# skitzoid/Box2D-MT

Hardware: AMD Instinct MI355X
Metric: world steps/sec at 99858 bodies per GPU (BASELINE config 3: Tumbler 100k, CCD off; Step = collide + island solve + broad-phase + state read-back); for N > 1: container-steps/s = world steps/s x N containers in the one sharded world (higher is better)
Workload: dtype f32

## Files before the change

### box2d-mt_amd/csrc/b2d_scan.h

```cpp
#ifndef B2D_SCAN_H
#define B2D_SCAN_H

#include <hip/hip_runtime.h>
#include <stdint.h>

#define SCAN_THREADS 256
#define SCAN_ITEMS 4
#define SCAN_TILE (SCAN_THREADS * SCAN_ITEMS)
#define SCAN_CHAIN_MAX_TILES 256
#define SCAN_ITEMS_WIDE 16
#define SCAN_TILE_WIDE (SCAN_THREADS * SCAN_ITEMS_WIDE)

__device__ __forceinline__ int scanAdd(int a, int b) { return a + b; }
__device__ __forceinline__ int4 scanAdd(int4 a, int4 b) { return make_int4(a.x + b.x, a.y + b.y, a.z + b.z, a.w + b.w); }
__device__ __forceinline__ void scanZero(int& a) { a = 0; }
__device__ __forceinline__ void scanZero(int4& a) { a = make_int4(0, 0, 0, 0); }
__device__ __forceinline__ void scanStoreAgent(int* p, int v) { __hip_atomic_store(p, v, __ATOMIC_RELAXED, __HIP_MEMORY_SCOPE_AGENT); }
__device__ __forceinline__ int scanLoadAgent(const int* p) { return __hip_atomic_load(p, __ATOMIC_RELAXED, __HIP_MEMORY_SCOPE_AGENT); }
__device__ __forceinline__ void scanStoreAgent(int4* p, int4 v)
{
	typedef int i4 __attribute__((ext_vector_type(4)));
	i4 q;
	q.x = v.x; q.y = v.y; q.z = v.z; q.w = v.w;
	asm volatile("global_store_dwordx4 %0, %1, off sc1\n\ts_nop 1" :: "v"(p), "v"(q) : "memory");
// ... 348 lines not shown
			unsigned long long m = __ballot(valid && ((d >> b) & 1));
			peers &= ((d >> b) & 1) ? m : ~m;
		}
		if (!valid) peers = 0;
		unsigned long long lower = peers & ((1ull << lane) - 1ull);
		int rankInWave = __popcll(lower);
		const bool first = valid && lower == 0;
		const int groupSize = __popcll(peers);
		if (first) waveCount[wave][d] = groupSize;
		__syncthreads();
		int total = 0;
		if (valid)
		{
			int off = digitBase[d];
			for (int w = 0; w < wave; ++w) off += waveCount[w][d];
			int dst = off + rankInWave;
			keysOut[dst] = key;
			valsOut[dst] = valR[k];
			if (first) total = waveCount[0][d] + waveCount[1][d] + waveCount[2][d] + waveCount[3][d];
		}
		__syncthreads();
		if (first)
		{
			bool lowest = true;
			for (int w = 0; w < wave; ++w) lowest = lowest && waveCount[w][d] == 0;
			if (lowest) digitBase[d] += total;
		}
		__syncthreads();
		if (first) waveCount[wave][d] = 0;
		__syncthreads();
	}
}

#endif
```

### box2d-mt_amd/csrc/b2hip_api_callbacks.h

```cpp

int b2hip_set_contact_filter(b2hip_world* w, b2hip_should_collide_fn fn, void* user)
{
	if (int rcu = checkUsable(w, "b2hip_set_contact_filter", true)) return rcu;
	w->filterFn = fn;
	w->filterUser = user;
	w->dw.userFilter = hasFilter(w) ? 1 : 0;
	return B2HIP_OK;
}

int b2hip_set_contact_filter_batch(b2hip_world* w, b2hip_should_collide_batch_fn fn, void* user)
{
	if (int rcu = checkUsable(w, "b2hip_set_contact_filter_batch", true)) return rcu;
	w->filterBatchFn = fn;
	if (fn) w->filterUser = user;
	w->dw.userFilter = hasFilter(w) ? 1 : 0;
	return B2HIP_OK;
}

int b2hip_default_should_collide(b2hip_world* w, int fixture_a, int fixture_b)
{
	if (!w || fixture_a < 0 || fixture_b < 0 || fixture_a >= (int)w->fixtures.size() || fixture_b >= (int)w->fixtures.size())
		return setError(B2HIP_ERR_INVALID, "bad fixture id");
	const HostFixture& a = w->fixtures[fixture_a];
	const HostFixture& b = w->fixtures[fixture_b];
// ... 154 lines not shown
	HIP_TRY(hipStreamSynchronize(w->stream));
	const void* src = nullptr;
	size_t elem = 16;
	switch (which)
	{
	case 0: src = w->b_pos.p; break;
	case 1: src = w->b_vel.p; break;
	case 2: src = w->li_bodies.p; elem = 4; break;
	case 3: src = w->b_force.p; break;
	case 4: src = w->b_flags.p; elem = 4; break;
	case 5: src = w->b_damp.p; break;
	case 6: src = w->b_mass.p; break;
	case 7: src = w->d_state.p; elem = 4; break;
	case 8: src = w->dbgPreVel.p; break;
	case 9: src = w->dbgVel.p; break;
	case 10: src = w->dbgLi.p; elem = 4; break;
	case 11: src = w->gridBar.p; elem = 4; break;
	case 12:
	{
		if (first < 0 || count < 0 || first + count > COLOR_SLOT_PADDED) return setError(B2HIP_ERR_INVALID, "colour census: [0, 65)");
		HIP_TRY(hipStreamSynchronize(w->stream));
		if (count > 0) HIP_TRY(hipMemcpy2D(out, sizeof(int), w->colorCount.p + colorSlot(first), COLOR_SLOT_STRIDE * sizeof(int), sizeof(int), (size_t)count, hipMemcpyDeviceToHost));
		return 0;
	}
	case 13: src = w->bodyColorMask.p; elem = 8; break;
	case 14: src = w->deg.p; elem = 4; break;
	case 15: src = w->hubList.p; elem = 4; break;
	case 16: src = w->bodyActive.p; elem = 8; break;
	case 17: src = w->b_blk1.p; elem = 4; break;
	case 18: src = w->li_ref.p; break;
	case 19: src = w->rowColor.p; elem = 4; break;
	case 20: src = w->blkRowStart.p; elem = 4; break;
	case 21: src = w->bodyRest.p; elem = 8; break;
	default: return setError(B2HIP_ERR_INVALID, "bad array id");
	}
	HIP_TRY(hipMemcpy(out, (const char*)src + (size_t)first * elem, (size_t)count * elem, hipMemcpyDeviceToHost));
	return 0;
}

int b2hip_debug_trace(b2hip_world* w, int index, char* label, int label_cap, uint64_t* hash)
{
	if (!w) return setError(B2HIP_ERR_INVALID, "null world");
	if (index < 0 || index >= (int)w->trace.size()) return 1;
	if (label && label_cap > 0)
	{
		strncpy(label, w->trace[index].first.c_str(), (size_t)label_cap - 1);
		label[label_cap - 1] = 0;
	}
	if (hash) *hash = w->trace[index].second;
	return 0;
}

int b2hip_get_profile(b2hip_world* w, float ms[13])
{
	if (!w || !ms) return setError(B2HIP_ERR_INVALID, "null argument");
	memcpy(ms, w->profile, sizeof(float) * 13);
	return 0;
}

int b2hip_get_counters(b2hip_world* w, b2hip_counters* out)
{
	if (!w || !out) return setError(B2HIP_ERR_INVALID, "null argument");
	memset(out, 0, sizeof(*out));
	out->bodies = (int)w->bodies.size();
	out->proxies = (int)w->fixtures.size();
	out->contacts = w->last.nContacts;
	out->touching_contacts = w->last.nTouching;
	out->islands = w->last.nIslands;
	out->small_islands = w->last.nSIslands;
	out->large_islands = w->last.nLIslands;
// ... 86 lines not shown
```

### box2d-mt_amd/csrc/b2hip_api_world.h

```cpp


const char* b2hip_last_error(void)
{
	return g_lastError.c_str();
}

const char* b2hip_version(void)
{
	return "b2hip 0.1 (gfx950)";
}

int b2hip_world_create(const b2hip_world_def* def, b2hip_world** out)
{
	if (!def || !out) return setError(B2HIP_ERR_INVALID, "null argument");
	int count = 0;
	hipError_t e = hipGetDeviceCount(&count);
	if (e != hipSuccess || count <= 0)
	{
		return setError(B2HIP_ERR_NO_DEVICE, "no HIP device available: the b2hip Step() path has no CPU fallback");
	}
	int current = 0;
	if (hipGetDevice(&current) != hipSuccess) current = 0;
	const int device = def->device >= 0 ? def->device : current;
	if (device >= count) return setError(B2HIP_ERR_NO_DEVICE, "no such HIP device");
// ... 166 lines not shown
	w->p_fat.release(); w->p_body.release(); w->p_shape.release(); w->p_key.release(); w->p_filter0.release(); w->p_filter1.release();
	w->p_mat.release(); w->d_shapes.release();
	for (int k = 0; k < 2; ++k)
	{
		w->c_ids[k].release(); w->c_key[k].release(); w->c_flags[k].release(); w->c_mat[k].release(); w->c_man0[k].release();
		w->c_man1[k].release(); w->c_imp[k].release(); w->c_man3[k].release(); w->c_color[k].release();
	}
	w->ht_keys.release(); w->d_joints.release(); w->d_gears.release(); w->li_ref.release();
	w->jadjStart.release(); w->jadj.release(); w->rootJointStart.release(); w->rootJointCursor.release();
	w->lj_list.release(); w->rootJointOkay.release();
	w->parent.release(); w->rootSeed.release(); w->rootBodies.release(); w->rootContacts.release(); w->rootJoints.release();
	w->rootIsland.release(); w->deg.release(); w->adjStart.release(); w->adjCursor.release(); w->adj.release(); w->adjSlot.release();
	w->rootScanIn.release(); w->rootScanOut.release();
	w->si_root.release(); w->si_bodyStart.release(); w->si_contactStart.release(); w->si_wStart.release(); w->si_maxLevel.release();
	w->si_bodies.release(); w->si_contacts.release(); w->si_level.release(); w->si_stack.release(); w->si_lastLevel.release();
	w->b_slot.release(); w->b_island.release(); w->chunkFirst.release();
	w->li_bodies.release(); w->li_contacts.release(); w->li_roots.release(); w->li_color.release(); w->colorCount.release();
	w->colorStart.release(); w->colorCursor.release(); w->li_sorted.release(); w->bodyClaim.release(); w->rootPen.release();
	w->bodyActive.release(); w->bodyRest.release(); w->b_posv.release(); w->evKey.release(); w->evInfo.release(); w->uncolList.release(); w->compactList.release(); w->gridBar.release(); w->hubRowOf.release(); w->hubList.release(); w->hubDelta.release(); w->hubMeta.release(); w->hubFirst.release(); w->solveSnapBody.release(); w->solveSnapImp.release(); w->solveSnapCFlags.release(); w->solveSnapJoints.release(); w->solveSnapGears.release();
	w->b_proxyHead.release(); w->p_next.release(); w->toiList.release(); w->toiPos2c.release(); w->toiDestroyList.release(); w->toiNewList.release();
	w->b_toiGroup.release(); w->toiGroups.release(); w->toiGroupCount.release(); w->toiGroupList.release(); w->toiMoved.release(); w->toiNew.release(); w->toiParent.release(); w->toiDomOf.release(); w->toiDomRoot.release(); w->toiDomCount.release(); w->toiDomBase.release(); w->toiDomFill.release(); w->toiDomFailed.release(); w->toiDomEvents.release(); w->toiDomList.release(); w->toiHull.release(); w->snapBody.release(); w->snapFat.release();
	w->c_mgr[0].release(); w->c_mgr[1].release(); w->dbgPreVel.release(); w->dbgVel.release(); w->dbgLi.release();
	w->rootSleepMin.release(); w->bodyColorMask.release(); w->rootDone.release(); w->lc.release(); w->warmDelta.release();
	w->moveBuf.release(); w->gridCount.release(); w->gridStart.release(); w->gridCursor.release(); w->gridItems.release(); w->gridFat.release(); w->arriveTree.release();
	w->largeProxies.release(); w->largeMoves.release(); w->pairKey.release(); w->pairKey2.release(); w->pairProxy.release(); w->pairProxy2.release();
	w->filterPairs.release();
	w->d_editOps.release();
	w->b_order.release(); w->orderBody.release(); w->bigRoots.release();
	w->pre_o0.release(); w->pre_o1.release(); w->pre_oimp.release(); w->pre_o3.release(); w->preRecs.release();
	w->postRecs.release(); w->filterList.release(); w->hostList.release(); w->toiLog.release(); w->toiVerdict.release();
	w->b_blk1.release(); w->b_adopt.release(); w->b_adoptStage.release(); w->blkRows.release(); w->blkRowStart.release(); w->blkCursor.release(); w->blkBodyCount.release(); w->blkBodyCursor.release();
	w->blkBodyStart.release(); w->blkBodies.release(); w->rowColor.release(); w->b_cutv.release();
	w->pairFirst.release(); w->pairRank.release(); w->scanTmp.release(); w->radixHist.release(); w->radixHistScan.release();
	w->keepFlag.release(); w->keepScan.release(); w->scanTmp4.release(); w->scanFlags.release(); w->stateOut.release(); w->consts.release();
	w->qIn.release(); w->qCounts.release(); w->qOffsets.release(); w->qItems.release(); w->qFlags.release(); w->qScanWork.release();
	w->qScanWords.release(); w->qWords.release(); w->qHits.release(); w->qDistances.release(); w->qPoses.release(); w->qShapes.release();
	w->qKeys.release(); w->qKeysWork.release(); w->qAny.release();
	if (w->qPinned) (void)hipHostFree(w->qPinned);
	if (w->h_state) (void)hipHostFree(w->h_state);
	if (w->h_dstate) (void)hipHostFree(w->h_dstate);
	if (w->h_pub) (void)hipHostFree(w->h_pub);
	if (w->h_pub2) (void)hipHostFree(w->h_pub2);
	if (w->h_solverWord) (void)hipHostFree(w->h_solverWord);
	for (int i = 0; i < 13; ++i)
		if (w->ev[i]) (void)hipEventDestroy(w->ev[i]);
	for (size_t i = 0; i < w->ktEvents.size(); ++i) (void)hipEventDestroy(w->ktEvents[i]);
	if (w->stream) (void)hipStreamDestroy(w->stream);
	if (w->stream2) (void)hipStreamDestroy(w->stream2);
	if (w->evFork) (void)hipEventDestroy(w->evFork);
	if (w->evJoin) (void)hipEventDestroy(w->evJoin);
	delete w;
}

int b2hip_set_gravity(b2hip_world* w, float gx, float gy)
{
	if (int rcu = checkUsable(w, "b2hip_set_gravity", true)) return rcu;
	if (!w) return setError(B2HIP_ERR_INVALID, "null world");
	w->def.gravity_x = gx;
	w->def.gravity_y = gy;
	return 0;
}

int b2hip_set_flags(b2hip_world* w, int allow_sleep, int warm_starting, int continuous, int sub_stepping)
{
	if (int rcu = checkUsable(w, "b2hip_set_flags", true)) return rcu;
	if (!w) return setError(B2HIP_ERR_INVALID, "null world");
	w->def.allow_sleep = allow_sleep;
// ... 1157 lines not shown
```

### box2d-mt_amd/csrc/b2hip_host_phases.h

```cpp

static int spExchangeState(b2hip_world* w, int mode);
static int spExchangePairs(b2hip_world* w, long long* totalPairs, int* straddling);
static int spResolve(b2hip_world* w, int nVirt = 0);
static int spAfterToi(b2hip_world* w);
static int spBeginStep(b2hip_world* w);

static int radixBits(int maxKey)
{
	int bits = 1;
	while ((1 << bits) <= maxKey && bits < 31) ++bits;
	return bits;
}

static void radixPasses(int first, int bits, std::vector<std::pair<int, int>>& out)
{
	const int passes = (bits + RADIX_BITS - 1) / RADIX_BITS;
	for (int p = 0, at = 0; p < passes; ++p)
	{
		const int width = (bits - at + (passes - p) - 1) / (passes - p);
		out.push_back(std::make_pair(first + at, width));
		at += width;
	}
}

static int radixSort(b2hip_world* w, uint64_t*& kin, uint64_t*& kout, int2*& vin, int2*& vout, const int* nPtr, int tilesCap, const std::vector<std::pair<int, int>>& passes, int overflowBit = 0)
{
	DW& d = w->dw;
	LAUNCH(w, k_radix_count, 1, 1, nPtr, 0, w->consts.p + 2, tilesCap, overflowBit ? &d.st->c.overflow : (int*)nullptr, overflowBit);
	for (size_t p = 0; p < passes.size(); ++p)
	{
		LAUNCH(w, k_radix_hist, tilesCap, RADIX_THREADS, kin, d.radixHist, nPtr, 0, passes[p].first, passes[p].second, tilesCap);
		deviceExclusiveScan<int>(w->stream, d.radixHist, w->radixHistScan.p, d.scanTmp, w->scanCtx, w->consts.p + 2, RADIX_DIGITS * tilesCap);
		LAUNCH(w, k_radix_scatter, tilesCap, RADIX_THREADS, kin, vin, kout, vout, w->radixHistScan.p, nPtr, 0, passes[p].first, passes[p].second);
		std::swap(kin, kout);
		std::swap(vin, vout);
	}
	return 0;
}

template <typename K>
static int applyHostList(b2hip_world* w, K kernel, const std::vector<int>& list)
{
	if (list.empty()) return 0;
	HIP_TRY(hipMemcpyAsync(w->hostList.p, list.data(), list.size() * sizeof(int), hipMemcpyHostToDevice, w->stream));
	LAUNCH(w, kernel, gridFor(list.size()), 256, w->dw, (const int*)w->hostList.p, (int)list.size());
	HIP_TRY(hipStreamSynchronize(w->stream));
	return 0;
}

static void askFilter(b2hip_world* w, const std::vector<int>& pairs2, std::vector<int>& verdict)
{
	const int n = (int)pairs2.size() / 2;
	verdict.assign((size_t)n, 1);
	if (n == 0) return;
	if (w->filterBatchFn) w->filterBatchFn(w->filterUser, n, pairs2.data(), verdict.data());
	else for (int i = 0; i < n; ++i) verdict[i] = w->filterFn(w->filterUser, pairs2[2 * i], pairs2[2 * i + 1]) ? 1 : 0;
}

static int userFilterPairs(b2hip_world* w, const int2* proxies)
{
// ... 1360 lines not shown
```

### box2d-mt_amd/csrc/b2hip_host_world.h

```cpp

static thread_local std::string g_lastError;

static int setError(int code, const std::string& msg)
{
	g_lastError = msg;
	return code;
}

#define HIP_TRY(expr)                                                                                   \
	do                                                                                                  \
	{                                                                                                   \
		hipError_t _e = (expr);                                                                         \
		if (_e != hipSuccess)                                                                           \
		{                                                                                               \
			return setError(B2HIP_ERR_HIP, std::string(#expr) + ": " + hipGetErrorString(_e));          \
		}                                                                                               \
	} while (0)

static void (*g_rcclDestroy)(void* comm) = nullptr;

template <typename T>
struct DevArray
{
	T* p = nullptr;
// ... 179 lines not shown
	int spIdle[6] = {0, 0, 0, 0, 0, 0};
	DevArray<int> spStraddle, spCount, spTarget, spSend, spRecv;
	std::vector<uint8_t> spOwners;
	bool spOwnersDirty = false;
	float spBounds[SHARD_MAX_RANKS + 1] = {0};
	b2hip_all_gather_fn gatherFn = nullptr;
	void* gatherUser = nullptr;
	int* spHost = nullptr;
	const int* spSendWiped = nullptr;
	int* spHdrHost = nullptr;
	int* spHdrDev = nullptr;
	int spHdrSeq = 0;
	int* spOwnHost = nullptr;
	int* spOwnDev = nullptr;
	size_t spOwnCapRows = 0;
	size_t spHostWords = 0;
	int spPairCap = 2048, spToiBodyCap = 256, spToiProxyCap = 512;
	int spOwned[SHARD_MAX_RANKS] = {0}, spOwnedProxies[SHARD_MAX_RANKS] = {0};
	long long spMigratedTotal = 0, spResolves = 0, spPairsSent = 0;
	size_t spBytesStep = 0;
	int spContactsBeforeToi = 0, spToiOrderBefore = 0, spTailCap = 64;
	int spToiUnsafe = 0;
	bool spToiSettled = false;
	DevArray<int4> spTailKey;
	DevArray<int2> spVirt;
	bool spTapeRecord = false;
	std::vector<std::pair<int*, size_t> > spTape;
	b2hip_world* spTapeFrom = nullptr;
	size_t spTapeCursor = 0;
	long long spToiRedos = 0;
	size_t spUp = 0;
	DevArray<int> scanFlags;
	ScanFlags scanCtx;
	DevArray<float> stateOut;
	DevArray<int> gridBar;
	int dfEpoch;
	bool noSideStream, profileDetail;
	int collideStage = -1;
	int solidRoundsEnv = 0;
	int collideSplitEnv = -1;
	bool collideUniOff = false;
	int collideSortEnv = -1;
	hipStream_t stream2 = nullptr;
	hipEvent_t evFork = nullptr, evJoin = nullptr;
	DevArray<int> consts;
	DevArray<unsigned long long> filterPairs;
	std::vector<int> nonStatic;
	bool orderDirty = false;
	DevArray<int> b_order, orderBody;
	DevArray<int> bigRoots;
	std::vector<int2> editOps;
	std::vector<int> proxyEdits;
	std::vector<int> fatEdits;
	bool proxyListsStale = false;
	DevArray<int2> d_editOps;
	b2hip_should_collide_fn filterFn = nullptr;
	void* filterUser = nullptr;
	bool refilterPending = false;
	b2hip_pre_solve_fn preSolveFn = nullptr;
	b2hip_pre_solve_batch_fn preSolveBatchFn = nullptr;
	b2hip_should_collide_batch_fn filterBatchFn = nullptr;
	void* preSolveUser = nullptr;
	bool postSolveOn = false;
	std::vector<b2hip_contact_impulse> postSolve;
	DevArray<float4> pre_o0, pre_o1, pre_oimp;
	DevArray<int4> pre_o3;
// ... 440 lines not shown
static int awaitColors(b2hip_world* w)
{
	if (int rc = pollPublished(w, (volatile const int*)&w->h_pub2->pubSeq, w->pubSeq2, "colour state")) return rc;
	memcpy(w->h_dstate, w->h_pub2, offsetof(DState, pubSeq));
	return 0;
}

static int awaitCensus(b2hip_world* w)
{
	if (w->pollDelayUs > 0) std::this_thread::sleep_for(std::chrono::microseconds(w->pollDelayUs));
	if (int rc = pollPublished(w, (volatile const int*)&w->h_pub->pubSeq, w->pubSeq, "island census")) return rc;
	memcpy(w->h_dstate, w->h_pub, offsetof(DState, pubSeq));
	return 0;
}

static bool envSet(const char* k) { return getenv(k) != nullptr; }
static bool envOn(const char* k) { const char* e = getenv(k); return e && atoi(e); }
static int envInt(const char* k, int unset) { const char* e = getenv(k); return e ? atoi(e) : unset; }

static void readSwitches(b2hip_world* w)
{
	DW& d = w->dw;
	w->debugSync = envSet("B2HIP_DEBUG");
	w->traceLaunches = envSet("B2HIP_TRACE_LAUNCHES");
	w->debugTrace = envSet("B2HIP_TRACE");
	w->forceLarge = envInt("B2HIP_FORCE_LARGE", 0);
	w->kernelTimingLaunches = envSet("B2HIP_SOLVER_LAUNCHES");
	w->noSideStream = envSet("B2HIP_NO_SIDE_STREAM");
	w->profileDetail = envInt("B2HIP_PROFILE_DETAIL", 1) != 0;
	if (const char* e = getenv("B2HIP_SOLID_ROUNDS")) { const int v = atoi(e); w->solidRoundsEnv = (v == 1 || v == 2 || v == 4 || v == 8) ? v : 0; }
	w->collideSplitEnv = envInt("B2HIP_COLLIDE_SPLIT", -1);
	w->collideUniOff = envInt("B2HIP_COLLIDE_UNI", 1) == 0;
	w->collideSortEnv = envInt("B2HIP_COLLIDE_SORT", -1);
	w->collideStage = envInt("B2HIP_COLLIDE_STAGE", -1);
	w->noSweepBlocks = envSet("B2HIP_NO_SWEEP_BLOCKS");
	w->tracePartition = envSet("B2HIP_TRACE_PARTITION");
	w->traceRecovery = envSet("B2HIP_TRACE_RECOVERY");
	if (const char* e = getenv("B2HIP_GRID_HALF")) { w->gridForced = true; w->gridHalf = atoi(e) != 0; d.gridHalf = w->gridHalf ? 1 : 0; }
	d.noChainCreate = envSet("B2HIP_TOI_NO_CHAIN_CREATE") ? 1 : 0;
	d.noOwnIdBlocks = envSet("B2HIP_NO_OWN_ID_BLOCKS") ? 1 : envSet("B2HIP_OWN_ID_BLOCKS_ALL") ? -1 : 0;
	w->noBlocks = envSet("B2HIP_NO_BLOCKS");
	w->blockLanes = 0;
	if (const char* e = getenv("B2HIP_BLOCK_LANES")) w->blockLanes = atoi(e) == 512 ? 512 : (atoi(e) == 256 ? 256 : (atoi(e) == 1024 ? 1024 : 0));
	w->toiSerialOnly = envSet("B2HIP_TOI_SERIAL");
	w->toiSyncOnly = envSet("B2HIP_TOI_SYNC");
	w->toiDomWideOnly = envSet("B2HIP_TOI_DOM_WIDE");
	w->noToiSpecDomains = envSet("B2HIP_TOI_NO_SPEC_DOMAINS");
	w->debugAssumeFreshGrid = envSet("B2HIP_DEBUG_ASSUME_FRESH_GRID");
	w->toiNoDomains = envSet("B2HIP_TOI_NO_DOMAINS");
	w->toiWhy = envSet("B2HIP_TOI_WHY");
	w->handoverWhy = envSet("B2HIP_HANDOVER_WHY");
	w->shardTrace = envOn("B2HIP_SHARD_TRACE");
	w->recoverOn = !envOn("B2HIP_NO_RECOVER");
	w->noCensusPoll = envOn("B2HIP_NO_CENSUS_POLL");
	w->noStatePoll = envOn("B2HIP_NO_STATE_POLL");
	w->lazyReadback = envOn("B2HIP_LAZY_READBACK");
	w->earlyRowsMin = envInt("B2HIP_EARLY_ROWS_MIN", w->earlyRowsMin);
	w->stepDeadlineS = getenv("B2HIP_STEP_DEADLINE_S") ? atof(getenv("B2HIP_STEP_DEADLINE_S")) : 300.0;
	w->pollDelayUs = envInt("B2HIP_TEST_POLL_DELAY_US", 0);
	d.bigChunks = envSet("B2HIP_BIG_CHUNKS") ? 1 : 0;
	d.smallMaxW = TINY_ISLAND_MAX_W;
	if (const char* e = getenv("B2HIP_SMALL_MAX_W")) d.smallMaxW = std::max(1, std::min((int)SMALL_ISLAND_MAX_W, atoi(e)));
	d.noFreeBodies = envOn("B2HIP_NO_FREE_BODIES") ? 1 : 0;
	d.testMaxColors = envInt("B2HIP_TEST_MAX_COLORS", 0);
	d.testColorRounds = envInt("B2HIP_TEST_COLOR_ROUNDS", 0);
	d.testSpinMax = std::max(0, envInt("B2HIP_TEST_SPIN_MAX", 0));
// ... 51 lines not shown
			if (rc) return rc;
		}
	}
	ENS(parent, nb); ENS(rootSeed, nb); ENS(rootBodies, nb); ENS(rootContacts, nb); ENS(rootJoints, nb); ENS(rootIsland, nb);
	ENS(deg, nb + 1); ENS(adjStart, nb + 2); ENS(adjCursor, nb); ENS(adj, 2 * cc); ENS(adjSlot, cc);
	ENS(rootScanIn, nb + 1); ENS(rootScanOut, nb + 2);
	ENS(si_root, nb + 1); ENS(si_bodyStart, nb + 2); ENS(si_contactStart, nb + 2); ENS(si_wStart, nb + 2); ENS(si_maxLevel, nb + 1);
	ENS(si_bodies, nb); ENS(si_contacts, cc); ENS(si_level, cc); ENS(si_stack, nb); ENS(si_lastLevel, nb);
	ENS(b_slot, nb); ENS(b_island, nb); ENS(chunkFirst, (nb + cc) / (TINY_CHUNK_LANES / 2) + 4);
	ENS(li_bodies, nb); ENS(li_contacts, cc); ENS(li_roots, nb); ENS(li_color, cc);
	ENS(colorCount, cc + 2 + COLOR_SLOT_PADDED * COLOR_SLOT_STRIDE); ENS(colorStart, cc + 2); ENS(colorCursor, cc + 2 + COLOR_SLOT_PADDED * COLOR_SLOT_STRIDE); ENS(li_sorted, cc); ENS(li_ref, cc);
	ENS(bodyClaim, nb); ENS(bodyColorMask, nb); ENS(bodyActive, nb); ENS(bodyRest, nb); ENS(b_posv, nb); ENS(evKey, cc); ENS(evInfo, cc); ENS(uncolList, COLOR_SMALL_MAX); ENS(compactList, COLOR_SMALL_MAX); ENS(hubRowOf, cc); ENS(hubList, cc); ENS(hubDelta, cc); ENS(hubMeta, 8); ENS(hubFirst, nb); ENS(solveSnapBody, w->recoverOn ? 6 * nb : 1); ENS(solveSnapImp, w->recoverOn ? cc : 1); ENS(solveSnapCFlags, w->recoverOn ? cc : 1); ENS(rootPen, ROOT_PEN_SLOTS * nb); ENS(rootDone, nb); ENS(rootSleepMin, nb);
	if (w->lc.cap < (size_t)LC_WORDS * cc)
	{
		rc = w->lc.ensure((size_t)LC_WORDS * cc, s, false, false);
		if (rc) return rc;
	}
	if (w->warmDelta.cap < 4 * cc)
	{
		rc = w->warmDelta.ensure(4 * cc, s, false, false);
		if (rc) return rc;
	}
	ENS(moveBuf, 2 * np + 64);
	const size_t gridSize = (size_t)nextPow2(2 * np);
	ENS(gridCount, gridSize); ENS(gridStart, gridSize + 2); ENS(gridCursor, gridSize); ENS(gridItems, np); ENS(gridFat, np); ENS(arriveTree, (size_t)ARRIVE_SITES * TREE_WORDS); ENS(largeProxies, np); ENS(largeMoves, 2 * np + 64);
	ENS(pairKey, capPairs); ENS(pairKey2, capPairs); ENS(pairProxy, capPairs); ENS(pairProxy2, capPairs);
	ENS(pairFirst, capPairs + 1); ENS(pairRank, capPairs + 2);
	const size_t maxScanN = std::max(std::max(nb + 2, gridSize + 2), std::max(cc + 2, capPairs + 2));
	const size_t radixTiles = capPairs / RADIX_TILE + 2;
	ENS(radixHist, RADIX_DIGITS * radixTiles + 2); ENS(radixHistScan, RADIX_DIGITS * radixTiles + 4);
	ENS(scanTmp, 3 * (std::max(maxScanN, RADIX_DIGITS * radixTiles) / SCAN_TILE + 8));
	ENS(scanTmp4, 3 * (maxScanN / SCAN_TILE + 8));
	ENS(scanFlags, std::max(maxScanN, RADIX_DIGITS * radixTiles) / SCAN_TILE + 8);
	ENS(keepFlag, cc + 1); ENS(keepScan, cc + 2);
	ENS(toiList, cc); ENS(toiPos2c, cc); ENS(toiDestroyList, cc); ENS(toiNewList, TOI_NEW_LIST_MAX);
	ENS(b_toiGroup, nb); ENS(toiGroups, nb); ENS(toiGroupCount, std::min<size_t>(nb, TOI_GROUPS_MAX)); ENS(toiGroupList, std::min<size_t>(nb, TOI_GROUPS_MAX) * CHAIN_ADJ_MAX); ENS(toiMoved, TOI_MOVED_ALL_MAX); ENS(toiNew, 8 * TOI_NEWPAIR_MAX); ENS(toiParent, nb); ENS(toiDomOf, nb); ENS(toiDomRoot, TOI_DOMAINS_MAX); ENS(toiDomCount, TOI_DOMAINS_MAX); ENS(toiDomBase, TOI_DOMAINS_MAX); ENS(toiDomFill, TOI_DOMAINS_MAX); ENS(toiDomFailed, TOI_DOMAINS_MAX); ENS(toiDomEvents, TOI_DOMAINS_MAX); ENS(toiDomList, cc); ENS(toiHull, np); ENS(snapBody, 5 * nb); ENS(snapFat, np);
	{
		const size_t nPre = hasPreSolve(w) ? cc : 1, nPost = w->postSolveOn ? cc : 1, nFil = hasFilter(w) ? cc : 1;
		ENS(pre_o0, nPre); ENS(pre_o1, nPre); ENS(pre_oimp, nPre); ENS(pre_o3, nPre); ENS(preRecs, nPre);
		ENS(postRecs, nPost); ENS(filterList, nFil);
		ENS(toiLog, listenerOn(w) && w->def.continuous ? cc : 1);
		ENS(toiVerdict, hasPreSolve(w) && w->def.continuous ? cc : 1);
		ENS(hostList, std::max<size_t>(std::max(4 * nPre, nFil), hasFilter(w) ? capPairs : 1));
	}
	ENS(b_blk1, nb); ENS(b_adopt, nb); ENS(b_adoptStage, 3 * nb); ENS(blkRows, (size_t)(MAX_BLOCKS + 2) * BLK_SLOT); ENS(blkRowStart, MAX_BLOCKS + 2); ENS(blkCursor, (size_t)(MAX_BLOCKS + 2) * BLK_SLOT); ENS(blkBodyCount, (size_t)(MAX_BLOCKS + 2) * BLK_SLOT); ENS(blkBodyCursor, (size_t)(MAX_BLOCKS + 2) * BLK_SLOT);
	ENS(blkBodyStart, MAX_BLOCKS + 2); ENS(blkBodies, nb); ENS(rowColor, cc); ENS(b_cutv, nb);
	ENS(b_owner, w->spatial ? nb : 1); ENS(spNewOwner, w->spatial ? nb : 1); ENS(spAwake, w->spatial ? nb : 1); ENS(spStraddle, w->spatial ? std::max<size_t>(w->spStraddle.cap, 4096) : 1);
	ENS(spCount, w->spatial ? (size_t)SP_RESOLVE_MAX * SHARD_MAX_RANKS : 1); ENS(spTarget, w->spatial ? SP_RESOLVE_MAX : 1);
	ENS(spTailKey, w->spatial ? capContacts : 1); ENS(spVirt, w->spatial ? SP_TAIL_MAX + 1 : 1);
	ENS(stateOut, 12 * nb + sizeof(DState) / sizeof(float) + 4);
	ENS(consts, 16);
	ENS(gridBar, 32);
#undef ENS
	w->scanCtx.words = w->scanFlags.p;
	w->scanCtx.count = w->scanFlags.cap;
	w->scanCtx.abortWord = &w->d_state.p->c.overflow;
	if (w->h_stateCap < 12 * nb + sizeof(DState) / sizeof(float) + 4)
	{
		ensureRows(w);
		float* old = w->h_state;
		w->h_state = nullptr;
		w->h_stateCap = 12 * nb * 2 + sizeof(DState) / sizeof(float) + 4;
		HIP_TRY(hipHostMalloc((void**)&w->h_state, w->h_stateCap * sizeof(float), hipHostMallocMapped | hipHostMallocCoherent));
		HIP_TRY(hipHostGetDevicePointer((void**)&w->d_hstate, w->h_state, 0));
		if (old)
		{
			memcpy(w->h_state, old, w->stateCount * 10 * sizeof(float));
			(void)hipHostFree(old);
		}
	}

	DW& d = w->dw;
	d.st = w->d_state.p;
	d.nBodies = (int)w->bodies.size();
	d.nProxies = (int)w->fixtures.size();
	d.nJoints = (int)w->joints.size();
	d.nShapes = (int)w->shapes.size();
	d.capContacts = (int)cc;
	d.capPairs = (int)w->pairKey.cap;
	d.capMoves = (int)w->moveBuf.cap;
	d.htMask = (uint32_t)(w->ht_keys.cap - 1);
	d.gridMask = (uint32_t)(gridSize - 1);
	d.b_pos = w->b_pos.p; d.b_pos0 = w->b_pos0.p; d.b_vel = w->b_vel.p; d.b_xf = w->b_xf.p; d.b_mass = w->b_mass.p;
	d.b_damp = w->b_damp.p; d.b_force = w->b_force.p; d.b_flags = w->b_flags.p; d.b_wake = w->b_wake.p; d.b_rowDirty = w->b_rowDirty.p;
	d.b_order = w->b_order.p; d.orderBody = w->orderBody.p; d.bigRoots = w->bigRoots.p;
	d.p_fat = w->p_fat.p; d.p_body = w->p_body.p; d.p_shape = w->p_shape.p; d.p_key = w->p_key.p;
	d.p_filter0 = w->p_filter0.p; d.p_filter1 = w->p_filter1.p; d.p_mat = w->p_mat.p; d.shapes = w->d_shapes.p;
	for (int k = 0; k < 2; ++k)
	{
// ... 383 lines not shown
```

### include/b2hip.h

```cpp
#ifndef B2HIP_H
#define B2HIP_H

#include <stddef.h>
#include <stdint.h>

#ifdef __cplusplus
extern "C" {
#endif

typedef struct b2hip_world b2hip_world;

typedef enum b2hip_status
{
	B2HIP_OK = 0,
	B2HIP_ERR_INVALID = -1,
	B2HIP_ERR_HIP = -2,
	B2HIP_ERR_NO_DEVICE = -3,
	B2HIP_ERR_UNSUPPORTED = -4,
	B2HIP_ERR_CAPACITY = -5
} b2hip_status;

enum { B2HIP_STATIC_BODY = 0, B2HIP_KINEMATIC_BODY = 1, B2HIP_DYNAMIC_BODY = 2 };
enum { B2HIP_SHAPE_CIRCLE = 0, B2HIP_SHAPE_EDGE = 1, B2HIP_SHAPE_POLYGON = 2,
       B2HIP_SHAPE_CHAIN = 3 };
// ... 353 lines not shown
int b2hip_shard_import(b2hip_world* w, const void* all_slabs, size_t stride_words);
int b2hip_shard_unique_id(void* id128);
int b2hip_shard_connect(b2hip_world* w, const void* id128, int rank, int count);
int b2hip_shard_exchange_bytes(b2hip_world* w, size_t* bytes);

typedef int (*b2hip_all_gather_fn)(void* user, const void* send, size_t bytes, void* recv);
typedef struct b2hip_shard_stats
{
	int32_t rank, count;
	int32_t owned_bodies, owned_proxies;
	int32_t owned_contacts;
	int32_t islands_solved;
	int32_t constraint_rows;
	int64_t migrated_bodies;
	int64_t resolutions;
	int64_t bytes_received_last_step;
	int64_t pairs_sent;
	int64_t toi_redos;
} b2hip_shard_stats;
int b2hip_shard_spatial(b2hip_world* w, int rank, int count, const uint8_t* owners);
int b2hip_set_shard_gather(b2hip_world* w, b2hip_all_gather_fn fn, void* user);
int b2hip_get_shard_stats(b2hip_world* w, b2hip_shard_stats* out);
int b2hip_shard_tape(b2hip_world* w, int mode, b2hip_world* from);
int b2hip_get_own_body_states(b2hip_world* w, int cap, int32_t* ids, b2hip_body_state* out);
int b2hip_get_body_owners(b2hip_world* w, int cap, uint8_t* owners);

int b2hip_get_island_labels(b2hip_world* w, int cap, int32_t* out);
int b2hip_get_fat_aabb(b2hip_world* w, int fixture, float out4[4]);
int b2hip_get_fat_aabbs(b2hip_world* w, int first, int count, float* out4n);

int b2hip_debug_hash(b2hip_world* w, int which, uint64_t* out);
int b2hip_debug_trace(b2hip_world* w, int index, char* label, int label_cap, uint64_t* hash);
int b2hip_debug_read(b2hip_world* w, int which, int first, int count, void* out);

int b2hip_save_snapshot(b2hip_world* w, void* buffer, size_t cap, size_t* needed);
int b2hip_load_snapshot(const void* buffer, size_t size, int device, b2hip_world** out);

int b2hip_set_lazy_readback(b2hip_world* w, int enable);

int b2hip_get_profile(b2hip_world* w, float ms[13]);
int b2hip_get_counters(b2hip_world* w, b2hip_counters* out);

int b2hip_get_solver_timing(b2hip_world* w, float* ms, double* algorithmic_bytes, int* constraints, int* bodies);

int b2hip_set_kernel_timing(b2hip_world* w, int enable);
int b2hip_set_kernel_timing_units(b2hip_world* w, long long units_a, long long units_b);
int b2hip_get_kernel_timing(b2hip_world* w, char* name, int name_cap, float* total_ms, int* launches, double* algorithmic_bytes);

typedef struct b2hip_query_filter
{
	uint16_t mask;
	int include_sensors;
} b2hip_query_filter;
typedef struct b2hip_query_item
{
	int32_t fixture, body;
} b2hip_query_item;
typedef struct b2hip_ray_hit
{
	int32_t fixture, body;
	float point_x, point_y, normal_x, normal_y, fraction;
	int32_t pad;
} b2hip_ray_hit;
#define B2HIP_QUERY_MAX (1 << 24)
int b2hip_query_aabbs(b2hip_world* w, int n, const float* boxes4n, const b2hip_query_filter* f, int cap, int32_t* offsets,
                      b2hip_query_item* items);
// ... 50 lines not shown
```

Baseline: 349.8.

## Add onesweep-style single-pass radix sort with decoupled look-back and fused histograms

Replaces the multi-kernel per-pass radix sort (count, histogram scan, scatter) with a prepare kernel that builds the histograms for every pass in one read. That is followed by one kernel per pass that ranks keys inside the tile and finds global digit offsets through a grouped decoupled look-back over epoch-tagged counters. This aims to cut kernel launches and extra global passes in the broad-phase and pair sorts. The change adds spin-waiting between tiles, with an abort path, and falls back to the old path during graph capture or when the tile count is too large. It also adds a test entry point and sort counters.

```diff
diff --git a/box2d-mt_amd/csrc/b2d_scan.h b/box2d-mt_amd/csrc/b2d_scan.h
--- a/box2d-mt_amd/csrc/b2d_scan.h
+++ b/box2d-mt_amd/csrc/b2d_scan.h
@@ -404,4 +404,266 @@
 	}
 }
 
+#define RADIX_MAX_PASSES 6
+#define RADIX_GROUP 16
+#define RADIX_ONEPASS_MAX_TILES 1024
+#define RADIX_PREPARE_TILES 2
+
+struct RadixLayout
+{
+	int passes;
+	int shift[RADIX_MAX_PASSES];
+	int width[RADIX_MAX_PASSES];
+};
+
+__global__ __launch_bounds__(RADIX_THREADS) void k_radix_prepare(const uint64_t* __restrict__ keys, const int* nPtr, int tilesCap, RadixLayout lay,
+	int* __restrict__ hist, int* __restrict__ histNext, int* overflow, int overflowBit)
+{
+	__shared__ int lh[RADIX_MAX_PASSES][RADIX_DIGITS];
+	for (int q = blockIdx.x * RADIX_THREADS + threadIdx.x; q < RADIX_MAX_PASSES * RADIX_DIGITS; q += gridDim.x * RADIX_THREADS) histNext[q] = 0;
+	int n = *nPtr;
+	if (n <= 0) return;
+	int numTiles = (n + RADIX_TILE - 1) / RADIX_TILE;
+	if (numTiles > tilesCap)
+	{
+		if (overflow != nullptr && blockIdx.x == 0 && threadIdx.x == 0) atomicOr(overflow, overflowBit);
+		numTiles = tilesCap;
+		n = numTiles * RADIX_TILE;
+	}
+	const int base = blockIdx.x * (RADIX_PREPARE_TILES * RADIX_TILE);
+	if (base >= n) return;
+	for (int p = 0; p < lay.passes; ++p)
+		for (int q = threadIdx.x; q < (1 << lay.width[p]); q += RADIX_THREADS) lh[p][q] = 0;
+	__syncthreads();
+	const int lane = threadIdx.x & 63;
+	for (int k = 0; k < RADIX_PREPARE_TILES * RADIX_ITEMS; ++k)
+	{
+		const int i = base + k * RADIX_THREADS + threadIdx.x;
+		const bool valid = i < n;
+		const uint64_t key = valid ? keys[i] : 0;
+		const int nValid = __popcll(__ballot(valid));
+		for (int p = 0; p < lay.passes; ++p)
+		{
+			const int d = valid ? (int)((uint32_t)(key >> lay.shift[p]) & ((1u << lay.width[p]) - 1u)) : -1;
+			const int prev = __shfl_up(d, 1);
+			const bool head = valid && (lane == 0 || prev != d);
+			const unsigned long long heads = __ballot(head);
+			if (head)
+			{
+				const unsigned long long rest = lane < 63 ? heads >> (lane + 1) : 0ull;
+				const int end = rest ? lane + __ffsll((long long)rest) : nValid;
+				atomicAdd(&lh[p][d], end - lane);
+			}
+		}
+	}
+	__syncthreads();
+	for (int p = 0; p < lay.passes; ++p)
+		for (int q = threadIdx.x; q < (1 << lay.width[p]); q += RADIX_THREADS)
+		{
+			const int v = lh[p][q];
+			if (v) atomicAdd(&hist[p * RADIX_DIGITS + q], v);
+		}
+}
+
+__device__ __forceinline__ int radixAwait(const unsigned* p, unsigned word, unsigned tag, int* abortWord, bool& gaveUp)
+{
+	unsigned polls = 0;
+	while (!gaveUp && (word >> 16) != tag)
+	{
+		word = __hip_atomic_load(p, __ATOMIC_RELAXED, __HIP_MEMORY_SCOPE_AGENT);
+		if ((++polls & 0xfffu) == 0u)
+		{
+			if (polls >= SCAN_SPIN_MAX) atomicOr(abortWord, SCAN_ABORT_BIT);
+			gaveUp = (__hip_atomic_load(abortWord, __ATOMIC_RELAXED, __HIP_MEMORY_SCOPE_AGENT) & SCAN_ABORT_BIT) != 0;
+		}
+	}
+	return (word >> 16) == tag ? (int)(word & 0xffffu) : 0;
+}
+
+__global__ __launch_bounds__(RADIX_THREADS) void k_radix_onepass(const uint64_t* __restrict__ keysIn, const int2* __restrict__ valsIn,
+	uint64_t* __restrict__ keysOut, int2* __restrict__ valsOut, const int* __restrict__ passHist, unsigned* counts, unsigned* groups,
+	const int* nPtr, int shift, int width, unsigned tag, int* abortWord)
+{
+	__shared__ int waveCount[4][RADIX_DIGITS];
+	__shared__ int digitBase[RADIX_DIGITS];
+	__shared__ int digitOff[RADIX_DIGITS];
+	__shared__ int scanLds[2 * SCAN_THREADS];
+	int n = *nPtr;
+	if (n <= 0) return;
+	int numTiles = (n + RADIX_TILE - 1) / RADIX_TILE;
+	if (numTiles > (int)gridDim.x) { numTiles = (int)gridDim.x; n = numTiles * RADIX_TILE; }
+	const int tile = blockIdx.x;
+	if (tile >= numTiles) return;
+	const int tid = threadIdx.x;
+	const int lane = tid & 63;
+	const int wave = tid >> 6;
+	const int D = 1 << width;
+	const uint32_t mask = (uint32_t)D - 1u;
+	const int base = tile * RADIX_TILE;
+	uint64_t keyR[RADIX_ITEMS];
+	int2 valR[RADIX_ITEMS];
+	int rank[RADIX_ITEMS];
+	const int first0 = base + wave * (RADIX_TILE / 4) + lane;
+#pragma unroll
+	for (int k = 0; k < RADIX_ITEMS; ++k)
+	{
+		const int i = first0 + k * 64;
+		keyR[k] = i < n ? keysIn[i] : 0;
+		valR[k] = i < n ? valsIn[i] : make_int2(0, 0);
+	}
+	for (int q = tid; q < D; q += RADIX_THREADS)
+	{
+		waveCount[0][q] = 0; waveCount[1][q] = 0; waveCount[2][q] = 0; waveCount[3][q] = 0;
+	}
+	{
+		constexpr int PER = RADIX_DIGITS / RADIX_THREADS;
+		int h[PER];
+		int sum = 0;
+#pragma unroll
+		for (int k = 0; k < PER; ++k)
+		{
+			const int q = tid * PER + k;
+			h[k] = q < D ? passHist[q] : 0;
+			sum += h[k];
+		}
+		int total;
+		int run = blockExclusiveScan(sum, &total, scanLds);
+#pragma unroll
+		for (int k = 0; k < PER; ++k)
+		{
+			const int q = tid * PER + k;
+			if (q < D) digitOff[q] = run;
+			run += h[k];
+		}
+	}
+	__syncthreads();
+	int* const myCount = waveCount[wave];
+#pragma unroll
+	for (int k = 0; k < RADIX_ITEMS; ++k)
+	{
+		const bool valid = first0 + k * 64 < n;
+		const int d = valid ? (int)((uint32_t)(keyR[k] >> shift) & mask) : -1;
+		unsigned long long peers = __ballot(valid);
+		for (int b = 0; b < width; ++b)
+		{
+			const unsigned long long m = __ballot(valid && ((d >> b) & 1));
+			peers &= ((d >> b) & 1) ? m : ~m;
+		}
+		if (!valid) peers = 0;
+		const unsigned long long lower = peers & ((1ull << lane) - 1ull);
+		const bool first = valid && lower == 0;
+		int before = 0;
+		if (first)
+		{
+			before = myCount[d];
+			myCount[d] = before + __popcll(peers);
+		}
+		before = __shfl(before, valid ? __ffsll((long long)peers) - 1 : lane);
+		rank[k] = before + __popcll(lower);
+	}
+	__syncthreads();
+	for (int q = tid; q < D; q += RADIX_THREADS)
+	{
+		const int c0 = waveCount[0][q], c1 = waveCount[1][q], c2 = waveCount[2][q], c3 = waveCount[3][q];
+		waveCount[0][q] = 0; waveCount[1][q] = c0; waveCount[2][q] = c0 + c1; waveCount[3][q] = c0 + c1 + c2;
+		digitBase[q] = c0 + c1 + c2 + c3;
+	}
+	for (int q = tid; q < D; q += RADIX_THREADS)
+		__hip_atomic_store(counts + (size_t)tile * D + q, (tag << 16) | (unsigned)digitBase[q], __ATOMIC_RELAXED, __HIP_MEMORY_SCOPE_AGENT);
+	bool gaveUp = false;
+	const int group = tile / RADIX_GROUP;
+	const int inGroup = tile - group * RADIX_GROUP;
+	for (int q0 = tid; q0 < D; q0 += 2 * RADIX_THREADS)
+	{
+		const bool two = q0 + RADIX_THREADS < D;
+		const unsigned* srcA = counts + (size_t)(group * RADIX_GROUP) * D + q0;
+		const unsigned* srcB = srcA + RADIX_THREADS;
+		unsigned wordA[RADIX_GROUP - 1], wordB[RADIX_GROUP - 1];
+#pragma unroll
+		for (int j = 0; j < RADIX_GROUP - 1; ++j)
+		{
+			wordA[j] = j < inGroup ? __hip_atomic_load(srcA + (size_t)j * D, __ATOMIC_RELAXED, __HIP_MEMORY_SCOPE_AGENT) : 0u;
+			wordB[j] = (two && j < inGroup) ? __hip_atomic_load(srcB + (size_t)j * D, __ATOMIC_RELAXED, __HIP_MEMORY_SCOPE_AGENT) : 0u;
+		}
+		int beforeA = 0, beforeB = 0;
+#pragma unroll
+		for (int j = 0; j < RADIX_GROUP - 1; ++j)
+			if (j < inGroup)
+			{
+				beforeA += radixAwait(srcA + (size_t)j * D, wordA[j], tag, abortWord, gaveUp);
+				if (two) beforeB += radixAwait(srcB + (size_t)j * D, wordB[j], tag, abortWord, gaveUp);
+			}
+		if (inGroup == RADIX_GROUP - 1)
+		{
+			unsigned* dstA = groups + (size_t)group * D + q0;
+			__hip_atomic_store(dstA, (tag << 16) | (unsigned)(beforeA + digitBase[q0]), __ATOMIC_RELAXED, __HIP_MEMORY_SCOPE_AGENT);
+			if (two) __hip_atomic_store(dstA + RADIX_THREADS, (tag << 16) | (unsigned)(beforeB + digitBase[q0 + RADIX_THREADS]), __ATOMIC_RELAXED, __HIP_MEMORY_SCOPE_AGENT);
+		}
+		digitOff[q0] += beforeA;
+		if (two) digitOff[q0 + RADIX_THREADS] += beforeB;
+	}
+	for (int q0 = tid; q0 < D; q0 += 2 * RADIX_THREADS)
+	{
+		const bool two = q0 + RADIX_THREADS < D;
+		int beforeA = 0, beforeB = 0;
+		for (int g0 = 0; g0 < group; g0 += 16)
+		{
+			const unsigned* srcA = groups + (size_t)g0 * D + q0;
+			const unsigned* srcB = srcA + RADIX_THREADS;
+			const int m = group - g0;
+			unsigned wordA[16], wordB[16];
+#pragma unroll
+			for (int j = 0; j < 16; ++j)
+			{
+				wordA[j] = j < m ? __hip_atomic_load(srcA + (size_t)j * D, __ATOMIC_RELAXED, __HIP_MEMORY_SCOPE_AGENT) : 0u;
+				wordB[j] = (two && j < m) ? __hip_atomic_load(srcB + (size_t)j * D, __ATOMIC_RELAXED, __HIP_MEMORY_SCOPE_AGENT) : 0u;
+			}
+#pragma unroll
+			for (int j = 0; j < 16; ++j)
+				if (j < m)
+				{
+					beforeA += radixAwait(srcA + (size_t)j * D, wordA[j], tag, abortWord, gaveUp);
+					if (two) beforeB += radixAwait(srcB + (size_t)j * D, wordB[j], tag, abortWord, gaveUp);
+				}
+		}
+		digitOff[q0] += beforeA;
+		if (two) digitOff[q0 + RADIX_THREADS] += beforeB;
+	}
+	__syncthreads();
+#pragma unroll
+	for (int k = 0; k < RADIX_ITEMS; ++k)
+	{
+		if (first0 + k * 64 < n)
+		{
+			const int d = (int)((uint32_t)(keyR[k] >> shift) & mask);
+			const int dst = digitOff[d] + myCount[d] + rank[k];
+			if ((unsigned)dst < (unsigned)n)
+			{
+				keysOut[dst] = keyR[k];
+				valsOut[dst] = valR[k];
+			}
+		}
+	}
+}
+
+struct RadixStatus
+{
+	unsigned* counts = nullptr;
+	unsigned* groups = nullptr;
+	size_t countsCap = 0, groupsCap = 0;
+	int* hist = nullptr;
+	int maxTiles = 0;
+	unsigned epoch = 0;
+	unsigned parity = 0;
+	int* abortWord = nullptr;
+};
+
+static inline bool radixOnepassFits(hipStream_t stream, const RadixStatus& rs, int tilesCap, size_t passes)
+{
+	if (rs.maxTiles <= 0 || tilesCap > rs.maxTiles || passes == 0 || passes > RADIX_MAX_PASSES) return false;
+	hipStreamCaptureStatus capturing = hipStreamCaptureStatusNone;
+	(void)hipStreamIsCapturing(stream, &capturing);
+	return capturing == hipStreamCaptureStatusNone;
+}
+
 #endif
diff --git a/box2d-mt_amd/csrc/b2hip_api_callbacks.h b/box2d-mt_amd/csrc/b2hip_api_callbacks.h
--- a/box2d-mt_amd/csrc/b2hip_api_callbacks.h
+++ b/box2d-mt_amd/csrc/b2hip_api_callbacks.h
@@ -210,10 +210,75 @@
 	case 19: src = w->rowColor.p; elem = 4; break;
 	case 20: src = w->blkRowStart.p; elem = 4; break;
 	case 21: src = w->bodyRest.p; elem = 8; break;
+	case 22:
+	{
+		const long long stats[2] = { w->statSorts, w->statSortsOnepass };
+		if (first < 0 || count < 0 || first + count > 2) return setError(B2HIP_ERR_INVALID, "pair-update statistics: [0, 2)");
+		memcpy(out, stats + first, (size_t)count * sizeof(long long));
+		return 0;
+	}
 	default: return setError(B2HIP_ERR_INVALID, "bad array id");
 	}
 	HIP_TRY(hipMemcpy(out, (const char*)src + (size_t)first * elem, (size_t)count * elem, hipMemcpyDeviceToHost));
 	return 0;
+}
+
+int b2hip_test_radix_sort(b2hip_world* w, int count, uint64_t* keys, int* payloads, int passes, const int* shifts, const int* widths)
+{
+	if (!w) return setError(B2HIP_ERR_INVALID, "null world");
+	DEVICE_GUARD(w);
+	if (count < 0 || passes < 1 || !shifts || !widths || (count > 0 && (!keys || !payloads))) return setError(B2HIP_ERR_INVALID, "bad argument");
+	if (w->stepActive) return setError(B2HIP_ERR_INVALID, "inside a step");
+	std::vector<std::pair<int, int>> lay;
+	for (int p = 0; p < passes; ++p)
+	{
+		if (widths[p] < 1 || widths[p] > RADIX_BITS || shifts[p] < 0 || shifts[p] + widths[p] > 64) return setError(B2HIP_ERR_INVALID, "bad pass");
+		lay.push_back(std::make_pair(shifts[p], widths[p]));
+	}
+	int rc = ensureCapacity(w, 0);
+	if (rc) return rc;
+	hipStream_t s = w->stream;
+	const int tilesCap = count / RADIX_TILE + 1;
+	const size_t tiles = (size_t)tilesCap + 1;
+	rc = w->radixHist.ensure(RADIX_DIGITS * tiles + 2, s); if (rc) return rc;
+	rc = w->radixHistScan.ensure(RADIX_DIGITS * tiles + 4, s); if (rc) return rc;
+	rc = w->scanTmp.ensure(3 * (RADIX_DIGITS * tiles / SCAN_TILE + 8), s); if (rc) return rc;
+	rc = w->scanFlags.ensure(RADIX_DIGITS * tiles / SCAN_TILE + 8, s); if (rc) return rc;
+	if (w->sortOnepass)
+	{
+		const size_t onepassTiles = std::min<size_t>(tiles, RADIX_ONEPASS_MAX_TILES);
+		rc = w->radixCounts.ensure(onepassTiles * RADIX_DIGITS, s, false); if (rc) return rc;
+		rc = w->radixGroups.ensure((onepassTiles / RADIX_GROUP + 1) * RADIX_DIGITS, s, false); if (rc) return rc;
+	}
+	rc = ensureCapacity(w, 0);
+	if (rc) return rc;
+	DevArray<uint64_t> k0, k1;
+	DevArray<int2> v0, v1;
+	DevArray<int> nDev;
+	const size_t room = (size_t)count + 1;
+	rc = k0.ensure(room, s, false, false);
+	if (!rc) rc = k1.ensure(room, s, false, false);
+	if (!rc) rc = v0.ensure(room, s, false, false);
+	if (!rc) rc = v1.ensure(room, s, false, false);
+	if (!rc) rc = nDev.ensure(1, s, false, true);
+	auto done = [&](int code) { (void)hipStreamSynchronize(s); k0.release(); k1.release(); v0.release(); v1.release(); nDev.release(); return code; };
+	if (rc) return done(rc);
+	hipError_t e = hipMemcpyAsync(nDev.p, &count, sizeof(int), hipMemcpyHostToDevice, s);
+	if (e == hipSuccess && count > 0) e = hipMemcpyAsync(k0.p, keys, (size_t)count * sizeof(uint64_t), hipMemcpyHostToDevice, s);
+	if (e == hipSuccess && count > 0) e = hipMemcpyAsync(v0.p, payloads, (size_t)count * sizeof(int2), hipMemcpyHostToDevice, s);
+	if (e != hipSuccess) return done(setError(B2HIP_ERR_HIP, hipGetErrorString(e)));
+	uint64_t *kin = k0.p, *kout = k1.p;
+	int2 *vin = v0.p, *vout = v1.p;
+	rc = radixSort(w, kin, kout, vin, vout, nDev.p, tilesCap, lay);
+	if (rc) return done(rc);
+	int overflow = 0;
+	e = hipMemcpyAsync(&overflow, &w->d_state.p->c.overflow, sizeof(int), hipMemcpyDeviceToHost, s);
+	if (e == hipSuccess && count > 0) e = hipMemcpyAsync(keys, kin, (size_t)count * sizeof(uint64_t), hipMemcpyDeviceToHost, s);
+	if (e == hipSuccess && count > 0) e = hipMemcpyAsync(payloads, vin, (size_t)count * sizeof(int2), hipMemcpyDeviceToHost, s);
+	if (e == hipSuccess) e = hipStreamSynchronize(s);
+	if (e != hipSuccess) return done(setError(B2HIP_ERR_HIP, hipGetErrorString(e)));
+	if (overflow & SCAN_ABORT_BIT) return done(setError(B2HIP_ERR_HIP, "a look-back of the sort gave up waiting for a predecessor tile"));
+	return done(0);
 }
 
 int b2hip_debug_trace(b2hip_world* w, int index, char* label, int label_cap, uint64_t* hash)
diff --git a/box2d-mt_amd/csrc/b2hip_api_world.h b/box2d-mt_amd/csrc/b2hip_api_world.h
--- a/box2d-mt_amd/csrc/b2hip_api_world.h
+++ b/box2d-mt_amd/csrc/b2hip_api_world.h
@@ -222,7 +222,7 @@
 	w->b_blk1.release(); w->b_adopt.release(); w->b_adoptStage.release(); w->blkRows.release(); w->blkRowStart.release(); w->blkCursor.release(); w->blkBodyCount.release(); w->blkBodyCursor.release();
 	w->blkBodyStart.release(); w->blkBodies.release(); w->rowColor.release(); w->b_cutv.release();
 	w->pairFirst.release(); w->pairRank.release(); w->scanTmp.release(); w->radixHist.release(); w->radixHistScan.release();
-	w->keepFlag.release(); w->keepScan.release(); w->scanTmp4.release(); w->scanFlags.release(); w->stateOut.release(); w->consts.release();
+	w->keepFlag.release(); w->keepScan.release(); w->scanTmp4.release(); w->scanFlags.release(); w->radixCounts.release(); w->radixGroups.release(); w->radixGlobalHist.release(); w->stateOut.release(); w->consts.release();
 	w->qIn.release(); w->qCounts.release(); w->qOffsets.release(); w->qItems.release(); w->qFlags.release(); w->qScanWork.release();
 	w->qScanWords.release(); w->qWords.release(); w->qHits.release(); w->qDistances.release(); w->qPoses.release(); w->qShapes.release();
 	w->qKeys.release(); w->qKeysWork.release(); w->qAny.release();
diff --git a/box2d-mt_amd/csrc/b2hip_host_phases.h b/box2d-mt_amd/csrc/b2hip_host_phases.h
--- a/box2d-mt_amd/csrc/b2hip_host_phases.h
+++ b/box2d-mt_amd/csrc/b2hip_host_phases.h
@@ -26,6 +26,39 @@
 static int radixSort(b2hip_world* w, uint64_t*& kin, uint64_t*& kout, int2*& vin, int2*& vout, const int* nPtr, int tilesCap, const std::vector<std::pair<int, int>>& passes, int overflowBit = 0)
 {
 	DW& d = w->dw;
+	w->statSorts += 1;
+	RadixStatus& rs = w->radixCtx;
+	if (w->sortOnepass && radixOnepassFits(w->stream, rs, tilesCap, passes.size()))
+	{
+		w->statSortsOnepass += 1;
+		if (rs.epoch + passes.size() > 0xffffu)
+		{
+			HIP_TRY(hipMemsetAsync(rs.counts, 0, rs.countsCap * sizeof(unsigned), w->stream));
+			HIP_TRY(hipMemsetAsync(rs.groups, 0, rs.groupsCap * sizeof(unsigned), w->stream));
+			rs.epoch = 0u;
+		}
+		RadixLayout lay;
+		lay.passes = (int)passes.size();
+		for (int p = 0; p < RADIX_MAX_PASSES; ++p)
+		{
+			lay.shift[p] = p < lay.passes ? passes[p].first : 0;
+			lay.width[p] = p < lay.passes ? passes[p].second : 0;
+		}
+		int* hist = rs.hist + rs.parity * (RADIX_MAX_PASSES * RADIX_DIGITS);
+		int* histNext = rs.hist + (1u - rs.parity) * (RADIX_MAX_PASSES * RADIX_DIGITS);
+		rs.parity = 1u - rs.parity;
+		LAUNCH(w, k_radix_prepare, (tilesCap + RADIX_PREPARE_TILES - 1) / RADIX_PREPARE_TILES, RADIX_THREADS, kin, nPtr, tilesCap, lay, hist, histNext,
+			overflowBit ? &d.st->c.overflow : (int*)nullptr, overflowBit);
+		for (size_t p = 0; p < passes.size(); ++p)
+		{
+			const unsigned tag = ++rs.epoch;
+			LAUNCH(w, k_radix_onepass, tilesCap, RADIX_THREADS, kin, vin, kout, vout, (const int*)(hist + p * RADIX_DIGITS), rs.counts, rs.groups, nPtr,
+				passes[p].first, passes[p].second, tag, rs.abortWord);
+			std::swap(kin, kout);
+			std::swap(vin, vout);
+		}
+		return 0;
+	}
 	LAUNCH(w, k_radix_count, 1, 1, nPtr, 0, w->consts.p + 2, tilesCap, overflowBit ? &d.st->c.overflow : (int*)nullptr, overflowBit);
 	for (size_t p = 0; p < passes.size(); ++p)
 	{
diff --git a/box2d-mt_amd/csrc/b2hip_host_world.h b/box2d-mt_amd/csrc/b2hip_host_world.h
--- a/box2d-mt_amd/csrc/b2hip_host_world.h
+++ b/box2d-mt_amd/csrc/b2hip_host_world.h
@@ -235,6 +235,11 @@
 	size_t spUp = 0;
 	DevArray<int> scanFlags;
 	ScanFlags scanCtx;
+	DevArray<unsigned> radixCounts, radixGroups;
+	DevArray<int> radixGlobalHist;
+	RadixStatus radixCtx;
+	bool sortOnepass = true;
+	long long statSorts = 0, statSortsOnepass = 0;
 	DevArray<float> stateOut;
 	DevArray<int> gridBar;
 	int dfEpoch;
@@ -741,6 +746,7 @@
 	w->collideSplitEnv = envInt("B2HIP_COLLIDE_SPLIT", -1);
 	w->collideUniOff = envInt("B2HIP_COLLIDE_UNI", 1) == 0;
 	w->collideSortEnv = envInt("B2HIP_COLLIDE_SORT", -1);
+	w->sortOnepass = envInt("B2HIP_SORT_ONEPASS", 1) != 0;
 	w->collideStage = envInt("B2HIP_COLLIDE_STAGE", -1);
 	w->noSweepBlocks = envSet("B2HIP_NO_SWEEP_BLOCKS");
 	w->tracePartition = envSet("B2HIP_TRACE_PARTITION");
@@ -858,6 +864,13 @@
 	ENS(scanTmp, 3 * (std::max(maxScanN, RADIX_DIGITS * radixTiles) / SCAN_TILE + 8));
 	ENS(scanTmp4, 3 * (maxScanN / SCAN_TILE + 8));
 	ENS(scanFlags, std::max(maxScanN, RADIX_DIGITS * radixTiles) / SCAN_TILE + 8);
+	const size_t onepassTiles = w->sortOnepass ? std::min<size_t>(radixTiles, RADIX_ONEPASS_MAX_TILES) : 0;
+	if (onepassTiles)
+	{
+		rc = w->radixCounts.ensure(onepassTiles * RADIX_DIGITS, s, false); if (rc) return rc;
+		rc = w->radixGroups.ensure((onepassTiles / RADIX_GROUP + 1) * RADIX_DIGITS, s, false); if (rc) return rc;
+		ENS(radixGlobalHist, 2 * RADIX_MAX_PASSES * RADIX_DIGITS);
+	}
 	ENS(keepFlag, cc + 1); ENS(keepScan, cc + 2);
 	ENS(toiList, cc); ENS(toiPos2c, cc); ENS(toiDestroyList, cc); ENS(toiNewList, TOI_NEW_LIST_MAX);
 	ENS(b_toiGroup, nb); ENS(toiGroups, nb); ENS(toiGroupCount, std::min<size_t>(nb, TOI_GROUPS_MAX)); ENS(toiGroupList, std::min<size_t>(nb, TOI_GROUPS_MAX) * CHAIN_ADJ_MAX); ENS(toiMoved, TOI_MOVED_ALL_MAX); ENS(toiNew, 8 * TOI_NEWPAIR_MAX); ENS(toiParent, nb); ENS(toiDomOf, nb); ENS(toiDomRoot, TOI_DOMAINS_MAX); ENS(toiDomCount, TOI_DOMAINS_MAX); ENS(toiDomBase, TOI_DOMAINS_MAX); ENS(toiDomFill, TOI_DOMAINS_MAX); ENS(toiDomFailed, TOI_DOMAINS_MAX); ENS(toiDomEvents, TOI_DOMAINS_MAX); ENS(toiDomList, cc); ENS(toiHull, np); ENS(snapBody, 5 * nb); ENS(snapFat, np);
@@ -881,6 +894,11 @@
 	w->scanCtx.words = w->scanFlags.p;
 	w->scanCtx.count = w->scanFlags.cap;
 	w->scanCtx.abortWord = &w->d_state.p->c.overflow;
+	w->radixCtx.counts = w->radixCounts.p; w->radixCtx.countsCap = w->radixCounts.cap;
+	w->radixCtx.groups = w->radixGroups.p; w->radixCtx.groupsCap = w->radixGroups.cap;
+	w->radixCtx.hist = w->radixGlobalHist.p;
+	w->radixCtx.maxTiles = w->sortOnepass ? (int)std::min<size_t>(std::min<size_t>(w->radixCounts.cap / RADIX_DIGITS, (w->radixGroups.cap / RADIX_DIGITS) * RADIX_GROUP), RADIX_ONEPASS_MAX_TILES) : 0;
+	w->radixCtx.abortWord = &w->d_state.p->c.overflow;
 	if (w->h_stateCap < 12 * nb + sizeof(DState) / sizeof(float) + 4)
 	{
 		ensureRows(w);
diff --git a/include/b2hip.h b/include/b2hip.h
--- a/include/b2hip.h
+++ b/include/b2hip.h
@@ -409,6 +409,7 @@
 int b2hip_debug_hash(b2hip_world* w, int which, uint64_t* out);
 int b2hip_debug_trace(b2hip_world* w, int index, char* label, int label_cap, uint64_t* hash);
 int b2hip_debug_read(b2hip_world* w, int which, int first, int count, void* out);
+int b2hip_test_radix_sort(b2hip_world* w, int count, uint64_t* keys, int* payloads, int passes, const int* shifts, const int* widths);
 
 int b2hip_save_snapshot(b2hip_world* w, void* buffer, size_t cap, size_t* needed);
 int b2hip_load_snapshot(const void* buffer, size_t size, int device, b2hip_world** out);
```

Result: faster. 356.1, median of 6 (+1.8%).
